# robocin/rSoccer

Measured on AMD Instinct MI355X. Metric: env-steps/sec (whole node), VSS-v0 3v3 @4096 envs, 1/2/4/8 GPU + CPU ref, higher is better.
Workload: dtype f32

## Files before the change

### __graft_entry__.py

```python
import os
import subprocess
import sys

ROOT = os.path.dirname(os.path.abspath(__file__))
if ROOT not in sys.path:
    sys.path.insert(0, ROOT)

CSRC = os.path.join(ROOT, "rsoccer_amd", "csrc")
HIP_SO = os.path.join(ROOT, "rsoccer_amd", "librsx_hip.so")
HIPCC_COMMON = ["--offload-arch=gfx950", "-O3", "-std=c++17", "-ffp-contract=off", "-fPIC",
                "-Wno-unused-value",
                "-mllvm", "-amdgpu-kernarg-preload-count=12",
                "-I" + os.path.join(ROOT, "include"), "-I" + CSRC]
HIP_UNITS = [
    ("rsx_api.hip", []),
    ("rsx_api_task.hip", []),
    ("rsx_api_ext.hip", []),
    ("rsx_lanes.hip", ["-mllvm", "-amdgpu-sched-strategy=max-ilp"]),
    ("rsx_epl.hip", ["-fno-slp-vectorize"]),
    ("rsx_big.hip", ["-fno-slp-vectorize"]),
    ("rsx_phys.hip", ["-mllvm", "-amdgpu-sched-strategy=max-ilp"]),
    ("rsx_sysid.hip", ["-mllvm", "-amdgpu-sched-strategy=max-ilp"]),
    ("rsx_plan.hip", ["-fno-slp-vectorize"]),
    ("rsx_plan_sampled.hip", ["-fno-slp-vectorize"]),
    ("rsx_policy.hip", ["-fno-slp-vectorize"]),
    ("rsx_render.hip", []),
    ("rsx_xfer.hip", []),
]

def _stale(target, sources):
    if not os.path.exists(target):
        return True
    t = os.path.getmtime(target)
# ... 79 lines not shown
```

### include/rsx.h

```cpp
#ifndef RSX_H
#define RSX_H

#include <stddef.h>
#include <stdint.h>

#ifdef __cplusplus
extern "C" {
#endif

#define RSX_ABI_VERSION 6
#define RSX_PHYSICS_MODEL 2

#define RSX_KIND_VSS 0
#define RSX_KIND_SSL 1

#define RSX_TASK_NONE                 0
#define RSX_TASK_VSS_V0               1
#define RSX_TASK_SSL_STATIC_DEFENDERS 2
#define RSX_TASK_SSL_DRIBBLING        3
#define RSX_TASK_SSL_CONTESTED        4
#define RSX_TASK_SSL_PASS_ENDURANCE   5
#define RSX_TASK_SSL_SCRIMMAGE         6
#define RSX_TASK_SSL_SCRIMMAGE_CROWDED 7

// ... 67 lines not shown
int rsx_step_dev(rsx_sim* h, void* stream);

int rsx_step_dev_flip(rsx_sim* h, void* stream);
int rsx_state_buffers(rsx_sim* h, float** current, float** other);
int rsx_reset_dev(rsx_sim* h, const float* ball_dev, const float* blue_dev, const float* yellow_dev,
                  const uint8_t* env_mask_dev, void* stream);

int rsx_step_dev_random(rsx_sim* h, int n, uint64_t seed, uint32_t first_tick, void* stream);


int rsx_task_attach(rsx_sim* h, int task, uint64_t seed, uint64_t env_id_base,
                    int max_episode_steps);
int rsx_task_view_get(rsx_sim* h, rsx_task_view* out);
int rsx_task_reseed(rsx_sim* h, uint64_t seed, void* stream);
int rsx_task_layout(rsx_sim* h, char* out, size_t n);
int rsx_task_placement_cache_stats(rsx_sim* h, int64_t out[2], void* stream);

int rsx_task_reset(rsx_sim* h, void* stream);
int rsx_task_reset_to(rsx_sim* h, const double* ball, const double* blue, const double* yellow,
                      const uint8_t* env_mask, void* stream);

int rsx_task_step(rsx_sim* h, const float* actions_dev, void* stream);
int rsx_task_step_n(rsx_sim* h, int n, void* stream);
int rsx_task_rollout(rsx_sim* h, int n, void* stream);

int rsx_task_enable_capture(rsx_sim* h, void* stream);
int rsx_drop_pending_hip_error(void);
int rsx_task_tick(rsx_sim* h, uint32_t* out, void* stream);

int rsx_task_lookahead(rsx_sim* h, const float* actions_dev, int n_candidates, int horizon, float gamma,
// ... 90 lines not shown
```

### rsoccer_amd/_lib.py

```python
import ctypes as C
import os

import numpy as np

_HERE = os.path.dirname(os.path.abspath(__file__))
LIB_PATH = os.environ.get("RSX_LIB") or os.path.join(_HERE, "librsx_hip.so")

KIND_VSS, KIND_SSL = 0, 1
TASK_NONE, TASK_VSS_V0, TASK_SSL_STATIC_DEFENDERS = 0, 1, 2
TASK_SSL_DRIBBLING, TASK_SSL_CONTESTED, TASK_SSL_PASS_ENDURANCE = 3, 4, 5
TASK_SSL_SCRIMMAGE, TASK_SSL_SCRIMMAGE_CROWDED = 6, 7
FIELD_KEYS = (
    "length", "width", "penalty_length", "penalty_width", "goal_width", "goal_depth",
    "ball_radius", "rbt_distance_center_kicker", "rbt_kicker_thickness", "rbt_kicker_width",
    "rbt_wheel0_angle", "rbt_wheel1_angle", "rbt_wheel2_angle", "rbt_wheel3_angle",
    "rbt_radius", "rbt_wheel_radius", "rbt_motor_max_rpm",
)
N_METRICS = 8
X_ROWS = 2
PHYSICS_PARAMS = ("m_robot", "m_ball", "e_rr", "e_rb", "e_wb", "e_wr", "mu_rr", "mu_rb", "mu_wb", "mu_g", "spin_dec",
                  "a_lin", "a_ang", "a_lat")
PHYSICS_COEFS = ("w_rb_r", "w_rb_b", "kt_rb_r", "kt_rb_b", "ope_rr", "ope_rb", "ope_wb", "e_wb", "e_wr", "mu_rr", "mu_rb", "mu_wb",
                 "a_lin_h", "a_lin_h2", "a_lat_h", "a_ang_h", "mu_g_dt", "spin_dec_dt")
PHYS_RAW, PHYS_COEF = 0, 1
TRACE_TERMS = ("ball_xy", "ball_v", "robot_xy", "robot_heading", "robot_v", "robot_omega")
METRIC_NAMES = ("env_steps", "episodes", "goals_for", "goals_against", "return_sum_q20",
                "episode_len_sum", "truncated_episodes", "reserved")

SYMBOLS = (
    "rsx_abi_version", "rsx_last_error", "rsx_device_count", "rsx_create", "rsx_destroy",
    "rsx_get_field_params", "rsx_reset", "rsx_step", "rsx_get_state", "rsx_step_state", "rsx_wire_buffers", "rsx_step_wire", "rsx_set_state",
    "rsx_get_state_full", "rsx_dev_view_get", "rsx_step_dev", "rsx_step_dev_random", "rsx_step_dev_flip", "rsx_state_buffers",
    "rsx_reset_dev", "rsx_task_attach",
    "rsx_task_view_get", "rsx_task_reseed", "rsx_task_layout", "rsx_task_placement_cache_stats", "rsx_task_reset", "rsx_task_reset_to", "rsx_task_step",
    "rsx_task_step_n", "rsx_task_rollout", "rsx_read_metrics", "rsx_metrics_fold", "rsx_check_finite",
    "rsx_task_checkpoint_size", "rsx_task_checkpoint_save", "rsx_task_checkpoint_load",
    "rsx_task_enable_capture", "rsx_task_tick", "rsx_drop_pending_hip_error", "rsx_task_lookahead",
    "rsx_physics_defaults", "rsx_physics_derive", "rsx_physics_enable", "rsx_physics_set", "rsx_physics_get",
    "rsx_physics_randomize", "rsx_physics_errors",
    "rsx_trace_load", "rsx_trace_eval",
    "rsx_render_view_reference", "rsx_render_size", "rsx_render_field", "rsx_render_open", "rsx_render", "rsx_render_errors",
    "rsx_task_transfer", "rsx_task_transfer_errors",
    "rsx_task_lookahead_sampled", "rsx_plan_candidates", "rsx_plan_update",
    "rsx_policy_num_params", "rsx_task_lookahead_policy",
)
ACT_RELU, ACT_TANH, ACT_CLIP = 0, 1, 2


class RsxError(RuntimeError):
# ... 54 lines not shown
    try:
        import torch
    except Exception:
        pass
    lib = C.CDLL(LIB_PATH)
    lib.rsx_last_error.restype = C.c_char_p
    vp, ip, dp = C.c_void_p, C.c_int, C.POINTER(C.c_double)
    lib.rsx_create.argtypes = [C.POINTER(vp), ip, ip, ip, ip, ip, ip, ip]
    lib.rsx_destroy.argtypes = [vp]
    lib.rsx_get_field_params.argtypes = [vp, dp]
    lib.rsx_reset.argtypes = [vp, vp, vp, vp, vp, vp]
    lib.rsx_step.argtypes = [vp, vp, vp]
    lib.rsx_get_state.argtypes = [vp, vp, vp]
    lib.rsx_step_state.argtypes = [vp, vp, vp, vp]
    lib.rsx_task_layout.argtypes = [vp, C.c_char_p, C.c_size_t]
    lib.rsx_task_placement_cache_stats.argtypes = [vp, C.POINTER(C.c_int64), vp]
    lib.rsx_set_state.argtypes = [vp, vp, vp]
    lib.rsx_wire_buffers.argtypes = [vp, C.POINTER(vp), C.POINTER(vp)]
    lib.rsx_step_wire.argtypes = [vp, vp]
    lib.rsx_get_state_full.argtypes = [vp, vp, vp]
    lib.rsx_dev_view_get.argtypes = [vp, C.POINTER(DevView)]
    lib.rsx_step_dev.argtypes = [vp, vp]
    lib.rsx_step_dev_random.argtypes = [vp, ip, C.c_uint64, C.c_uint32, vp]
    lib.rsx_step_dev_flip.argtypes = [vp, vp]
    lib.rsx_state_buffers.argtypes = [vp, C.POINTER(vp), C.POINTER(vp)]
    lib.rsx_reset_dev.argtypes = [vp, vp, vp, vp, vp, vp]
    lib.rsx_task_attach.argtypes = [vp, ip, C.c_uint64, C.c_uint64, ip]
    lib.rsx_task_view_get.argtypes = [vp, C.POINTER(TaskView)]
    lib.rsx_task_reseed.argtypes = [vp, C.c_uint64, vp]
    lib.rsx_task_reset.argtypes = [vp, vp]
# ... 229 lines not shown

    def task_attach(self, task, seed=0, env_id_base=0, max_episode_steps=0):
        _chk(self._lib.rsx_task_attach(self._h, task, seed, env_id_base, max_episode_steps))
        t = TaskView()
        _chk(self._lib.rsx_task_view_get(self._h, C.byref(t)))
        self._tview = t
        self.task = task
        self.obs_dim, self.act_dim, self.info_dim = t.obs_dim, t.act_dim, t.info_dim
        self.max_episode_steps = t.max_episode_steps

    def task_layout(self):
        buf = C.create_string_buffer(64)
        _chk(self._lib.rsx_task_layout(self._h, buf, 64))
        return buf.value.decode()

    def placement_cache_stats(self, stream=None):
        out = (C.c_int64 * 2)()
        _chk(self._lib.rsx_task_placement_cache_stats(self._h, out, self._stream(stream)))
        return int(out[0]), int(out[1])

    def task_tensors(self):
        t, B = self._tview, self.num_envs
        return dict(
            obs=self._tensor(t.obs, (B, t.obs_dim), "<f4"),
            reward=self._tensor(t.reward, (B,), "<f4"),
            terminated=self._tensor(t.terminated, (B,), "|u1"),
            truncated=self._tensor(t.truncated, (B,), "|u1"),
            info=self._rows(t.info, t.info_dim, t.row_stride),
            final_obs=self._tensor(t.final_obs, (B, t.obs_dim), "<f4"),
            steps=self._tensor(t.steps, (B,), "<i4"),
# ... 222 lines not shown
```

### rsoccer_amd/csrc/rsx_api_task.hip

```cpp
#include <cmath>
#include <cstdio>
#include <cstring>

#include "rsx_handle.hpp"
#include "rsx_math.hpp"
#include "rsx_plan_common.hpp"

using namespace rsx;

#ifndef RSX_PCACHE_MAX_ENVS
#define RSX_PCACHE_MAX_ENVS 16384
#endif

namespace {

int grid_for(const rsx_sim* h) { return lane_grid(h->L, h->P.num_envs); }
int helpers_for(const rsx_sim* h, int mode) { return mode == MODE_STEP && h->d_pcache && !h->d_phys ? (h->P.num_envs + 63) / 64 : 0; }

Layout stepping_layout(const rsx_sim* h, int mode) { return mode == MODE_STEP ? h->plan.step : mode == MODE_ROLLOUT ? h->plan.rollout : Layout::Lanes; }
int step_grid(const rsx_sim* h, int mode) {
    switch (stepping_layout(h, mode)) {
        case Layout::Epl: return epl_grid(h->P.num_envs);
        case Layout::Quad: return ssl_quad_grid(h->P.num_envs);
        default: return grid_for(h) + helpers_for(h, mode);
    }
}
void launch_task_of(const rsx_sim* h, const float* actions, int n_steps, int mode, hipStream_t s) {
    const Buffers b = buffers_of(h, mode == MODE_STEP ? actions : nullptr);
    const bool rollout = mode == MODE_ROLLOUT;
    switch (stepping_layout(h, mode)) {
        case Layout::Epl:
            if (h->P.task == RSX_TASK_VSS_V0) launch_vss_epl(rollout, h->P, b, n_steps, s); else launch_ssl_epl(h->P.task, rollout, h->P, b, n_steps, s);
            break;
        case Layout::Quad: launch_ssl_quad(h->P, b, n_steps, s); break;
        case Layout::LanesBig: launch_scrimmage_big(rollout, h->P, b, n_steps, s); break;
        case Layout::Lanes:
            if (h->d_phys) launch_task_phys(h->P, b, h->L, h->NR, h->d_phys, n_steps, mode, s);
            else launch_task(h->P, b, h->L, h->NR, helpers_for(h, mode), n_steps, mode, s);
            break;
    }
}
bool rollout_as_steps(const rsx_sim* h) { return h->plan.rollout_as_steps || (h->tick_dev && h->plan.step == Layout::Quad); }

}

void rsx::plan_stepping(rsx_sim* h) {
    const Params& P = h->P;
    h->plan = plan_layout(LayoutQuery{P.task, P.kind, h->L, h->NR, P.n_blue, P.num_envs, P.row_stride, P.state_dim, P.obs_dim, P.n_sub,
                                      h->d_phys != nullptr, std::getenv("RSX_LAYOUT")});
    h->tick_slots = step_grid(h, MODE_STEP);
}

extern "C" {

int rsx_task_attach(rsx_sim* h, int task, uint64_t seed, uint64_t env_id_base, int max_episode_steps) {
    RSX_ENTER(h);
    if (h->P.task != RSX_TASK_NONE) return fail(RSX_ERR_STATE, "a task is already attached");
    if (env_id_base > 0xFFFFFFFFull || env_id_base + (uint64_t)h->P.num_envs > 0x100000000ull)
        return fail(RSX_ERR_ARG, "env_id_base + num_envs exceeds 2^32 (global env ids are 32-bit)");
    Params P = h->P;
    if (derive_task(task, seed, env_id_base, max_episode_steps, h->M, P))
        return fail(RSX_ERR_ARG, "task does not match the simulator (VSS_V0: VSS, n_blue >= 1; STATIC_DEFENDERS: SSL 1vN; DRIBBLING: SSL 1v4; CONTESTED: SSL 1v1; PASS_ENDURANCE: SSL 2v0; SCRIMMAGE: SSL)");
    if (P.obs_dim > 64) return fail(RSX_ERR_ARG, "observation wider than 64 floats is not supported");
    if (task >= RSX_TASK_SSL_DRIBBLING && task <= RSX_TASK_SSL_PASS_ENDURANCE && h->L != 8)
// ... 89 lines not shown
    HIP_TRY(hipMemcpyAsync(out, h->d_pcstats, 2 * sizeof(int64_t), hipMemcpyDeviceToHost, (hipStream_t)stream));
    HIP_TRY(hipStreamSynchronize((hipStream_t)stream));
    return RSX_OK;
}

int rsx_task_layout(rsx_sim* h, char* out, size_t n) {
    if (!h || !out || n == 0) return fail(RSX_ERR_ARG, "null argument");
    if (h->P.task == RSX_TASK_NONE) return fail(RSX_ERR_STATE, "no task attached (rsx_task_attach)");
    const Layout lay = h->plan.step;
    const char* name = lay == Layout::Epl ? "one-lane-per-env" : lay == Layout::Quad ? "four-lanes-per-env" : lay == Layout::LanesBig ? "32-lanes-per-env-large-batch"
                     : h->L == 8 ? "8-lanes-per-env" : h->L == 16 ? "16-lanes-per-env" : h->L == 32 ? "32-lanes-per-env" : "64-lanes-per-env";
    std::snprintf(out, n, "%s", name);
    return RSX_OK;
}

int rsx_task_view_get(rsx_sim* h, rsx_task_view* out) {
    if (!h || !out) return fail(RSX_ERR_ARG, "null argument");
    if (h->P.task == RSX_TASK_NONE) return fail(RSX_ERR_STATE, "no task attached (rsx_task_attach)");
    const size_t B = (size_t)h->P.num_envs;
    out->task = h->P.task; out->obs_dim = h->P.obs_dim; out->act_dim = h->M.act_dim;
    out->info_dim = h->M.info_dim; out->max_episode_steps = h->P.max_steps;
    const size_t S = (size_t)h->P.row_stride;
    out->obs = h->d_obs; out->reward = h->d_aux + (size_t)ROW_REWARD * S;
    out->terminated = h->d_flags; out->truncated = h->d_flags + B;
    out->info = h->d_aux + (size_t)ROW_INFO * S; out->final_obs = h->d_final_obs;
    out->steps = (int32_t*)(h->d_aux + (size_t)ROW_STEPS * S); out->actions = h->d_actions;
    out->metrics = (int64_t*)h->d_metrics; out->row_stride = h->P.row_stride;
    return RSX_OK;
}

// ... 424 lines not shown
```

### rsoccer_amd/csrc/rsx_layout.hpp

```cpp
#pragma once
#include <algorithm>
#include <cstddef>
#include <cstring>

#include "rsx.h"
#include "rsx_params.hpp"

#ifndef RSX_EPL_MIN_ENVS
#define RSX_EPL_MIN_ENVS 98304
#endif
#ifndef RSX_EPL_MIN_ENVS_SSL
#define RSX_EPL_MIN_ENVS_SSL 65536
#endif
constexpr int RSX_EPL_MIN_ENVS_DRIBBLING = 49152, RSX_EPL_MIN_ENVS_DUEL = 32768;
#ifndef RSX_BIG_MIN_ENVS
#define RSX_BIG_MIN_ENVS 8192
#endif
#ifndef RSX_QUAD_MIN_ENVS
#define RSX_QUAD_MIN_ENVS 32768
#endif
#ifndef RSX_QUAD_MIN_ENVS_CROWDED
#define RSX_QUAD_MIN_ENVS_CROWDED 65536
#endif
#ifndef RSX_QUAD_ROLLOUT_MIN_ENVS
#define RSX_QUAD_ROLLOUT_MIN_ENVS 49152
#endif
#ifndef RSX_QUAD_ROLLOUT_MIN_ENVS_CROWDED
#define RSX_QUAD_ROLLOUT_MIN_ENVS_CROWDED 196608
#endif

namespace rsx {

enum class Layout { Lanes, LanesBig, Quad, Epl };

struct StepPlan {
    Layout step = Layout::Lanes;
    Layout rollout = Layout::Lanes;
    bool rollout_as_steps = false;
};

struct LayoutQuery {
    int task, kind, L, NR, n_blue, num_envs, row_stride, state_dim, obs_dim, n_sub;
    bool physics;
    const char* env_layout;
};

inline StepPlan plan_layout(const LayoutQuery& q) {
    StepPlan p;
    if (q.physics) return p;
    const auto asked = [&](const char* name) { return q.env_layout && std::strcmp(q.env_layout, name) == 0; };
    const int task = q.task, n_robots = (q.state_dim - 5) / (q.kind == RSX_KIND_VSS ? ModelD<RSX_KIND_VSS>::rs : ModelD<RSX_KIND_SSL>::rs);
    const size_t rows = (size_t)std::max(q.state_dim + X_ROWS, aux_rows(n_robots));
    const bool rows_below_2g = rows * (size_t)q.row_stride * sizeof(float) < ((size_t)1 << 31);
    if ((task == RSX_TASK_SSL_SCRIMMAGE || task == RSX_TASK_SSL_SCRIMMAGE_CROWDED) && q.NR == 22 && q.L == 32) {
        const bool spread = task == RSX_TASK_SSL_SCRIMMAGE;
        p.step = p.rollout = q.num_envs >= RSX_BIG_MIN_ENVS ? Layout::LanesBig : Layout::Lanes;
        const int quad_min = spread ? RSX_QUAD_MIN_ENVS : RSX_QUAD_MIN_ENVS_CROWDED;
        const bool fits = rows_below_2g && q.n_sub > 0 && q.n_blue == 11;
        if (fits && (q.env_layout ? asked("quad") : (quad_min > 0 && q.num_envs >= quad_min))) {
            p.step = Layout::Quad;
            p.rollout_as_steps = q.num_envs >= (spread ? RSX_QUAD_ROLLOUT_MIN_ENVS : RSX_QUAD_ROLLOUT_MIN_ENVS_CROWDED);
        }
        return p;
    }
    const bool fixed_ssl = task == RSX_TASK_SSL_DRIBBLING || task == RSX_TASK_SSL_CONTESTED || task == RSX_TASK_SSL_PASS_ENDURANCE;
    if ((task == RSX_TASK_VSS_V0 && q.NR == 6 && q.L == 8) || (task == RSX_TASK_SSL_STATIC_DEFENDERS && q.NR == 7 && q.L == 8) || fixed_ssl) {
        const int epl_min = task == RSX_TASK_VSS_V0 ? RSX_EPL_MIN_ENVS : task == RSX_TASK_SSL_STATIC_DEFENDERS ? RSX_EPL_MIN_ENVS_SSL
                          : task == RSX_TASK_SSL_DRIBBLING ? RSX_EPL_MIN_ENVS_DRIBBLING : RSX_EPL_MIN_ENVS_DUEL;
        const bool epl = asked("epl") || (!asked("lanes") && q.num_envs >= epl_min);
        if (epl && rows_below_2g && (size_t)q.num_envs * q.obs_dim * sizeof(float) < ((size_t)1 << 31)) p.step = p.rollout = Layout::Epl;
    }
    return p;
}

}
```

### rsoccer_amd/csrc/rsx_task_step_body.inc

```
    constexpr bool HOT = MODE != MODE_ROLLOUT;
    Params P = P_;
    Buffers bufs = bufs_;
    if (HOT) {
        RSX_UNPACK_HOT(P);
        bufs.state = hp_state; bufs.aux = hp_aux; bufs.actions = hp_in; bufs.flags = hp_flags;
    }
    const int n_steps_arg = hp_n_steps & RSX_N_STEPS_MASK;
    constexpr int mode = MODE == MODE_ROLLOUT ? MODE_STEP : MODE;
    const int n_steps = MODE == MODE_ROLLOUT ? n_steps_arg : 1;
    const bool tick_dev = __builtin_expect((hp_n_steps & RSX_TICK_DEV) != 0, 0);
    using K = KC<KIND>;
    using T = TC<TASK>;
    constexpr int G = 64 / L;
    constexpr int ID = T::info_dim;
    constexpr int AD = T::act_dim;
    __shared__ Shared<L> sh;
    constexpr bool PC = !PHYS && MODE == MODE_STEP && L == 8 && TASK == RSX_TASK_SSL_STATIC_DEFENDERS && NR == 7;
    if constexpr (PC) {
        if (__builtin_expect(bufs.pcache != nullptr && (int)blockIdx.x >= hp_per_xcd * 8, 0)) {
            const StepTick th = step_tick(tick_dev, P, bufs, 1u);
            if (th.ok) placement_helper<KIND, L, TASK, (PC ? NR : 1)>(P, bufs, (int)blockIdx.x - hp_per_xcd * 8, th.t, sh);
            return;
        }
    }
    StepTick tk{0u, true};
    if (MODE == MODE_STEP || MODE == MODE_ROLLOUT) {
        tk = step_tick(tick_dev, P, bufs, (uint32_t)n_steps);
        if (__builtin_expect(!tk.ok, 0)) return;
    }
    const uint32_t tick0 = tk.t;
    const int lane = threadIdx.x;
    const int b = LaneMap<L>::body(lane), g = LaneMap<L>::env(lane);
    const int tile = tile_of_block(HOT ? hp_per_xcd : (int)(gridDim.x >> 3));
    const int e = tile * G + g;
    const int N = NR ? NR : P.n_robots;
    const bool live = e < P.num_envs;
    const bool is_robot = live && b < N, is_ball = live && b == N;
    const size_t B = (size_t)P.num_envs;
    const uint32_t env_id = P.env_id_base + (uint32_t)e;
    constexpr int OD_C = obs_dim_c<TASK, NR>();
    const int OD = OD_C ? OD_C : P.obs_dim;
#define auxe(ROW) at_byte(bufs.aux, (ix_t)(ROW) * ((ix_t)4 * (ix_t)P.row_stride) + (ix_t)4 * (ix_t)e)

#ifdef RSX_TIMING
    if (lane == 0) { sh.dbg = bufs.dbg; bufs.dbg[(size_t)13 * gridDim.x + blockIdx.x] = __builtin_amdgcn_s_memrealtime(); }
#endif
    RSX_STAMP(0);
    Body o; float od, wd, wheels[4];
    const RawBody raw = load_raw<KIND>(P, bufs.state, e, b, is_robot, is_ball);
    constexpr bool CODE_PF = !PHYS && KIND == RSX_KIND_VSS && MODE == MODE_STEP;
    uint32_t code_touch = 0;
    if (CODE_PF) {
        unsigned long long pc;
        asm volatile("s_getpc_b64 %0" : "=s"(pc));
        code_touch = __builtin_nontemporal_load(reinterpret_cast<const uint32_t*>(reinterpret_cast<const char*>(pc) + 128u * (unsigned)lane));
    }
    std::conditional_t<PHYS, EnvCoef, LitCoef<KIND>> cf{};
    if constexpr (PHYS) if (live) load_coefs(P, phys, e, cf);
    int steps = 0; uint32_t episode = 0;
    if (live) {
        steps = __float_as_int(auxe(ROW_STEPS));
        episode = __float_as_uint(auxe(ROW_EPISODE));
    }
    float ou0 = 0.0f, ou1 = 0.0f;
    if (TASK == RSX_TASK_VSS_V0 && is_robot && b >= 1) {
        ou0 = auxe(ROW_OU + 2 * b); ou1 = auxe(ROW_OU + 2 * b + 1);
    }
    float info[10] = {0, 0, 0, 0, 0, 0, 0, 0, 0, 0};
    float prev_pot = 0.0f, ep_ret = 0.0f;
    if (is_ball) {
#pragma unroll
        for (int i = 0; i < ID; ++i)
            if (!(TASK == RSX_TASK_VSS_V0 && (i == 0 || i >= 4))) info[i] = auxe(ROW_INFO + i);
        prev_pot = auxe(ROW_PREV_POT);
        if (TASK != RSX_TASK_VSS_V0) ep_ret = auxe(ROW_EP_RET);
    }
    const bool counts_steps = (MODE == MODE_STEP || MODE == MODE_ROLLOUT) && blockIdx.x == 0 && lane == 0;
    unsigned long long steps_before = 0;
    if (counts_steps) steps_before = bufs.metrics[0];
    float reward = 0.0f; int term = 0, trunc = 0;
    bool success = false;
    bool against = false;
    bool was_reset = false;
    const bool fed = MODE == MODE_STEP && bufs.actions != nullptr;
    float act[AD];
#pragma unroll
    for (int i = 0; i < AD; ++i) act[i] = 0.0f;
    if (TASK == RSX_TASK_SSL_SCRIMMAGE) {
        if (fed && is_robot) {
#pragma unroll
            for (int i = 0; i < AD; ++i) act[i] = at_byte(bufs.actions, (ix_t)4 * (((ix_t)e * (ix_t)N + (ix_t)b) * (ix_t)AD + (ix_t)i));
// ... 5 lines not shown

    float pcx = 0.0f, pcy = 0.0f, pcth = 0.0f;
    uint32_t ptag = 0u;
    bool pc_on = false;
    if constexpr (PC) {
        pc_on = bufs.pcache != nullptr;
        if (pc_on && (is_robot || is_ball)) {
            constexpr int NBD = (PC ? NR : 1) + 1;
            const float* const pr = bufs.pcache + (size_t)((tick0 + 1u) & 1u) * (size_t)pcache_rows<NBD>() * B;
            pcx = pr[(size_t)(0 * NBD + b) * B + e]; pcy = pr[(size_t)(1 * NBD + b) * B + e]; pcth = pr[(size_t)(2 * NBD + b) * B + e];
            ptag = __float_as_uint(pr[(size_t)(3 * NBD) * B + e]);
        }
    }

    StepDraw pre;
    if (MODE == MODE_STEP) pre = draw_for_step<KIND, TASK>(P, env_id, tick0, b, is_robot, fed);

    __builtin_amdgcn_s_waitcnt(0x0F70);
    if (CODE_PF) asm volatile("" :: "v"(code_touch));
    interpret_body<KIND>(raw, is_robot, is_ball, o, od, wd, wheels);
    RSX_STAMP(1);

    for (int it = 0; it < n_steps; ++it) {
        bool ended;
        const float obs_ts = prev_pot;
        if (mode == 2) {
            const bool flagged = live && bufs.flags[2 * B + e] != 0;
            if (flagged) {
                episode += 1; steps = 0; ou0 = 0.0f; ou1 = 0.0f;
                if constexpr (PHYS) phys_redraw(P, phys, e, env_id, episode, b == 0, cf);
                if (is_ball) {
#pragma unroll
                    for (int i = 0; i < 10; ++i) info[i] = 0.0f;
#pragma unroll
                    for (int i = 0; i < ID; ++i) auxe(ROW_INFO + i) = 0.0f;
// ... 31 lines not shown
            physics<KIND, L, NR>(P, o, b, g, live, sh, cf);
            RSX_STAMP(3);
            if (MODE == MODE_STEP && KIND == RSX_KIND_SSL) {
                typedef const __attribute__((address_space(4))) uint32_t* kw_t;
                constexpr size_t KOFF = RSX_PARAMS_KERNARG_OFFSET;
                static_assert(sizeof(Params) % 4 == 0 && KOFF % 4 == 0, "parameter block in dwords");
                kw_t pk = (kw_t)__builtin_amdgcn_kernarg_segment_ptr() + KOFF / 4;
                asm volatile("" : "+s"(pk));
                struct Words { uint32_t w[sizeof(Params) / 4]; } raw;
#pragma unroll
                for (size_t i = 0; i < sizeof(Params) / 4; ++i) raw.w[i] = pk[i];
                P = __builtin_bit_cast(Params, raw);
                RSX_UNPACK_HOT(P);
            }

#include "rsx_step_wire.inc"
            write_obs<KIND, TASK>(P, bufs.obs + (size_t)e * OD, b, is_robot, is_ball, o.x, o.y, o.vx, o.vy, o.s, o.c, wd, o.ir, obs_ts);
#include "rsx_step_xr.inc"
            wave_sync();
            if (is_ball) {
                const float* xr = sh.x0[g];
                task_reward<KIND, TASK>(P, xr, o.x, o.y, lastx, lasty, first_step, prev_pot, info, reward, term, success, against);
                ep_ret = ep_ret + reward;
            }
            steps += 1;
            trunc = steps >= P.max_steps;
            const unsigned long long endm = __ballot(is_ball && (term | trunc));
            ended = live && ((endm >> (LaneMap<L>::slot(N, g))) & 1ull) != 0;
            if (is_ball) {
#pragma unroll
                for (int i = 0; i < ID; ++i)
                    if (!(TASK == RSX_TASK_VSS_V0 && (i == 0 || i >= 4)) || term || first_step) auxe(ROW_INFO + i) = info[i];
                auxe(ROW_REWARD) = reward;
                if (MODE == MODE_STEP) { bufs.flags[(ix_t)e] = (uint8_t)term; bufs.flags[(ix_t)P.num_envs + (ix_t)e] = (uint8_t)trunc; }
                else { bufs.flags[e] = (uint8_t)term; bufs.flags[B + e] = (uint8_t)trunc; }
            }
        }

        RSX_STAMP(4);
        if (RSX_RARE_B(KIND, 4, __any(ended))) {
            if (ended && mode == 0) {
                write_obs<KIND, TASK>(P, bufs.final_obs + (size_t)e * OD, b, is_robot, is_ball, o.x, o.y, o.vx, o.vy, o.s, o.c, wd, o.ir, obs_ts);
            }
            if (ended && mode == 0) episode += 1;
            if (KIND == RSX_KIND_VSS) {
                if (ended && is_ball && mode == 0) {
                    unsigned long long* const ms = metric_slot(bufs);
                    atomicAdd(&ms[1], 1ull);
                    if (info[4] > 0.0f) atomicAdd(&ms[2], 1ull);
                    if (info[5] > 0.0f) atomicAdd(&ms[3], 1ull);
                    atomicAdd(&ms[4], (unsigned long long)__float2ll_rn(vss_episode_return(info) * 1048576.0f));
                    atomicAdd(&ms[5], (unsigned long long)steps);
                    if (trunc && !term) atomicAdd(&ms[6], 1ull);
                }
            } else if (mode == 0) {
                static_assert(KIND == RSX_KIND_VSS || L >= 6, "metrics fan-out needs 6 lanes per env");
                uint32_t* const mv = reinterpret_cast<uint32_t*>(sh.x0[g]);
                if (ended && is_ball) {
                    unsigned long long inc[6];
                    inc[0] = 1ull;
                    inc[1] = success ? 1ull : 0ull;
                    inc[2] = against ? 1ull : 0ull;
                    inc[3] = (unsigned long long)__float2ll_rn(ep_ret * 1048576.0f);
                    inc[4] = (unsigned long long)steps;
                    inc[5] = (trunc && !term) ? 1ull : 0ull;
#pragma unroll
                    for (int k = 0; k < 6; ++k) { mv[2 * k] = (uint32_t)inc[k]; mv[2 * k + 1] = (uint32_t)(inc[k] >> 32); }
                }
                wave_sync();
// ... 47 lines not shown
            RSX_STAMP(18);
        }

        wave_sync();
    }

    RSX_STAMP(5);
    if (mode != 2) store_body<KIND>(P, bufs.state, e, b, is_robot, is_ball, o, od, wd, wheels, P.n_sub != 0 || was_reset);
    if (live && b == 0) {
        auxe(ROW_STEPS) = __int_as_float(steps);
        auxe(ROW_EPISODE) = __uint_as_float(episode);
    }
    if (TASK == RSX_TASK_VSS_V0 && is_robot && b >= 1) {
        auxe(ROW_OU + 2 * b) = ou0; auxe(ROW_OU + 2 * b + 1) = ou1;
    }
    if (is_ball) {
        auxe(ROW_PREV_POT) = prev_pot;
        if (TASK != RSX_TASK_VSS_V0) auxe(ROW_EP_RET) = ep_ret;
#undef auxe
    }
    if (counts_steps) bufs.metrics[0] = steps_before + (unsigned long long)P.num_envs * (unsigned long long)n_steps;
    RSX_STAMP(6);
#ifdef RSX_TIMING
    __builtin_amdgcn_s_waitcnt(0x0F70);
    RSX_STAMP(7);
    if (lane == 0) bufs.dbg[(size_t)14 * gridDim.x + blockIdx.x] = __builtin_amdgcn_s_memrealtime();
#endif
```

### rsoccer_amd/csrc/rsx_units.hpp

```cpp
#pragma once
#include <hip/hip_runtime.h>

#include <cstdint>

struct rsx_render_view;

namespace rsx {

struct Params;
struct Buffers;

void launch_sim(const Params& P, const Buffers& b, int L, int NR, float* state_out, int rand_tick, hipStream_t s);
void launch_task(const Params& P, const Buffers& b, int L, int NR, int helpers, int n_steps, int mode, hipStream_t s);
void launch_count_nonfinite(const float* p, size_t n, unsigned long long* out, hipStream_t s);
void launch_fold_metrics(unsigned long long* metrics, unsigned long long* slots, hipStream_t s);
void launch_reset_dev(float* st, const float* ball, const float* blue, const float* yellow, const uint8_t* mask, int B, int S, int rows,
                      int rs, int nb, int ny, float r_ball, hipStream_t s);
void launch_wire_cmds_in(const double* wire, float* cmds, unsigned B, unsigned NC, unsigned S, hipStream_t s);
void launch_wire_state_out(const float* st, double* wire, unsigned B, unsigned rows, unsigned S, hipStream_t s);
void launch_tick_fill(uint32_t* slots, int from, int to, uint32_t value, int copy, hipStream_t s);
#ifdef RSX_TIMING
inline unsigned long long* g_dbg = nullptr;
#endif
void launch_vss_epl(bool rollout, const Params& P, const Buffers& b, int n_steps, hipStream_t s);
void launch_ssl_epl(int task, bool rollout, const Params& P, const Buffers& b, int n_steps, hipStream_t s);
void launch_ssl_quad(const Params& P, const Buffers& b, int n_steps, hipStream_t s);
int epl_grid(int num_envs);
int ssl_quad_grid(int num_envs);
void launch_scrimmage_big(bool rollout, const Params& P, const Buffers& b, int n_steps, hipStream_t s);
void launch_task_phys(const Params& P, const Buffers& b, int L, int NR, float* phys, int n_steps, int mode, hipStream_t s);
void launch_sim_phys(const Params& P, const Buffers& b, int L, int NR, float* phys, float* state_out, int rand_tick, hipStream_t s);
void launch_phys_init(float* blk, int B, int S, int kind, int ts_ms, hipStream_t s);
void launch_phys_set(float* blk, const float* vals, const uint8_t* mask, int B, int S, int vstride, hipStream_t s);
void launch_phys_ranges(float* blk, const float* lo, const float* hi, uint32_t mask, hipStream_t s);
void launch_trace_eval(const Params& P, int L, int NR, const float* phys, float* state, float* loss, const float* frames,
                       const float* cmds, const int32_t* anchors, int n_frames, int n_anchors, int horizon, hipStream_t s);
long long lookahead_grid(int L, int num_envs, int n_candidates);
void launch_task_lookahead(const Params& P, int L, int NR, const float* state, const float* aux, const uint32_t* ticks, const float* phys,
                           const float* actions, int n_candidates, int horizon, float gamma, float* returns, int32_t* steps,
                           uint8_t* flags, float* last_obs, hipStream_t s);
struct PlanSampler;
void launch_task_lookahead_sampled(const Params& P, int L, int NR, const float* state, const float* aux, const uint32_t* ticks, const float* phys,
                                   const float* mean, const PlanSampler& S, int n_candidates, int horizon, float gamma, float* returns,
                                   int32_t* steps, uint8_t* flags, float* last_obs, hipStream_t s);
// ... 25 lines not shown
```

### rsoccer_amd/csrc/rsx_variants.hpp

```cpp
#pragma once
#include <type_traits>
#include <utility>

#include "rsx_launch.hpp"
#include "rsx_kernels.hpp"

namespace rsx {

template <int V> using int_c = std::integral_constant<int, V>;


template <int MAX_L, typename F>
void with_generic_variant(const int L, F&& f) {
    static_assert(MAX_L == 32 || MAX_L == 64, "widest lane group the unit instantiates");
    switch (L) {
        case 8: f(int_c<8>{}, int_c<0>{}); break;
        case 16: f(int_c<16>{}, int_c<0>{}); break;
        case 32: f(int_c<32>{}, int_c<0>{}); break;
        default: f(int_c<MAX_L>{}, int_c<0>{}); break;
    }
}

template <int KIND, int MAX_L, typename F>
void with_sim_variant(const int L, const int NR, F&& f) {
// ... 34 lines not shown
template <typename F>
void with_mode(const int mode, F&& f) {
    switch (mode) {
        case MODE_STEP: f(int_c<MODE_STEP>{}); break;
        case MODE_ROLLOUT: f(int_c<MODE_ROLLOUT>{}); break;
        case MODE_RESET: f(int_c<MODE_RESET>{}); break;
        default: f(int_c<MODE_REFRESH>{}); break;
    }
}
inline int mode_steps(const int mode, const int n_steps) { return mode == MODE_STEP || mode == MODE_ROLLOUT ? n_steps : 1; }

struct HotGrid {
    int tiles, helpers = 0;
    size_t lds = 0;
    int per_xcd = 0;
};

template <typename... KArgs, typename... Tail>
void launch_hot(void (*kernel)(KArgs...), const HotGrid& g, hipStream_t s, float* out, const float* in, const int n, const Params& P,
                const Buffers& b, Tail&&... tail) {
    rsx_launch(kernel, dim3((unsigned)(g.tiles + g.helpers)), dim3(64), g.lds, s, b.state, out, in, b.flags, P.num_envs,
               RSX_HOT_DIM(P.state_dim, P.row_stride, P.num_envs), g.per_xcd ? g.per_xcd : g.tiles >> 3, n, P, b, std::forward<Tail>(tail)...);
}
template <typename... KArgs, typename... Tail>
void launch_task_hot(void (*kernel)(KArgs...), const HotGrid& g, hipStream_t s, const int n_steps, const Params& P, const Buffers& b, Tail&&... tail) {
    launch_hot(kernel, g, s, b.aux, b.actions, n_steps, P, b, std::forward<Tail>(tail)...);
}
template <typename... KArgs, typename... Tail>
void launch_sim_hot(void (*kernel)(KArgs...), const HotGrid& g, hipStream_t s, float* state_out, const int rand_tick, const Params& P, const Buffers& b, Tail&&... tail) {
    launch_hot(kernel, g, s, state_out, b.cmds, rand_tick, P, b, std::forward<Tail>(tail)...);
}

}
```

Baseline: 436.2 million.

## Split VSS-v0 single step into paired physics and service wavefronts

Adds a 128-thread paired kernel for the VSS-v0 single-step path at small env counts. The second wavefront loads episode bookkeeping, draws the random actions, and later computes reward, flags and metrics from ball positions passed through LDS. The first wavefront runs physics and obs writes. The aim is to take the RNG draws, aux loads and reward tail off the critical physics wavefront, at the cost of LDS traffic and workgroup barriers.

New measurement: 448.9 million, median of 6. 1.03x the previous value.

```diff
diff --git a/__graft_entry__.py b/__graft_entry__.py
--- a/__graft_entry__.py
+++ b/__graft_entry__.py
@@ -17,6 +17,7 @@
     ("rsx_api_task.hip", []),
     ("rsx_api_ext.hip", []),
     ("rsx_lanes.hip", ["-mllvm", "-amdgpu-sched-strategy=max-ilp"]),
+    ("rsx_pair.hip", ["-mllvm", "-amdgpu-sched-strategy=max-ilp"]),
     ("rsx_epl.hip", ["-fno-slp-vectorize"]),
     ("rsx_big.hip", ["-fno-slp-vectorize"]),
     ("rsx_phys.hip", ["-mllvm", "-amdgpu-sched-strategy=max-ilp"]),
diff --git a/include/rsx.h b/include/rsx.h
--- a/include/rsx.h
+++ b/include/rsx.h
@@ -105,6 +105,7 @@
 int rsx_task_view_get(rsx_sim* h, rsx_task_view* out);
 int rsx_task_reseed(rsx_sim* h, uint64_t seed, void* stream);
 int rsx_task_layout(rsx_sim* h, char* out, size_t n);
+int rsx_task_service_wave(rsx_sim* h, int* out);
 int rsx_task_placement_cache_stats(rsx_sim* h, int64_t out[2], void* stream);
 
 int rsx_task_reset(rsx_sim* h, void* stream);
diff --git a/rsoccer_amd/_lib.py b/rsoccer_amd/_lib.py
--- a/rsoccer_amd/_lib.py
+++ b/rsoccer_amd/_lib.py
@@ -32,7 +32,7 @@
     "rsx_get_field_params", "rsx_reset", "rsx_step", "rsx_get_state", "rsx_step_state", "rsx_wire_buffers", "rsx_step_wire", "rsx_set_state",
     "rsx_get_state_full", "rsx_dev_view_get", "rsx_step_dev", "rsx_step_dev_random", "rsx_step_dev_flip", "rsx_state_buffers",
     "rsx_reset_dev", "rsx_task_attach",
-    "rsx_task_view_get", "rsx_task_reseed", "rsx_task_layout", "rsx_task_placement_cache_stats", "rsx_task_reset", "rsx_task_reset_to", "rsx_task_step",
+    "rsx_task_view_get", "rsx_task_reseed", "rsx_task_layout", "rsx_task_service_wave", "rsx_task_placement_cache_stats", "rsx_task_reset", "rsx_task_reset_to", "rsx_task_step",
     "rsx_task_step_n", "rsx_task_rollout", "rsx_read_metrics", "rsx_metrics_fold", "rsx_check_finite",
     "rsx_task_checkpoint_size", "rsx_task_checkpoint_save", "rsx_task_checkpoint_load",
     "rsx_task_enable_capture", "rsx_task_tick", "rsx_drop_pending_hip_error", "rsx_task_lookahead",
@@ -117,6 +117,7 @@
     lib.rsx_get_state.argtypes = [vp, vp, vp]
     lib.rsx_step_state.argtypes = [vp, vp, vp, vp]
     lib.rsx_task_layout.argtypes = [vp, C.c_char_p, C.c_size_t]
+    lib.rsx_task_service_wave.argtypes = [vp, C.POINTER(C.c_int)]
     lib.rsx_task_placement_cache_stats.argtypes = [vp, C.POINTER(C.c_int64), vp]
     lib.rsx_set_state.argtypes = [vp, vp, vp]
     lib.rsx_wire_buffers.argtypes = [vp, C.POINTER(vp), C.POINTER(vp)]
@@ -376,6 +377,11 @@
         _chk(self._lib.rsx_task_layout(self._h, buf, 64))
         return buf.value.decode()
 
+    def task_service_wave(self):
+        out = C.c_int(0)
+        _chk(self._lib.rsx_task_service_wave(self._h, C.byref(out)))
+        return bool(out.value)
+
     def placement_cache_stats(self, stream=None):
         out = (C.c_int64 * 2)()
         _chk(self._lib.rsx_task_placement_cache_stats(self._h, out, self._stream(stream)))
diff --git a/rsoccer_amd/csrc/rsx_api_task.hip b/rsoccer_amd/csrc/rsx_api_task.hip
--- a/rsoccer_amd/csrc/rsx_api_task.hip
+++ b/rsoccer_amd/csrc/rsx_api_task.hip
@@ -36,6 +36,7 @@
         case Layout::LanesBig: launch_scrimmage_big(rollout, h->P, b, n_steps, s); break;
         case Layout::Lanes:
             if (h->d_phys) launch_task_phys(h->P, b, h->L, h->NR, h->d_phys, n_steps, mode, s);
+            else if (mode == MODE_STEP && h->plan.service_wave) launch_task_pair(h->P, b, n_steps, s);
             else launch_task(h->P, b, h->L, h->NR, helpers_for(h, mode), n_steps, mode, s);
             break;
     }
@@ -47,7 +48,7 @@
 void rsx::plan_stepping(rsx_sim* h) {
     const Params& P = h->P;
     h->plan = plan_layout(LayoutQuery{P.task, P.kind, h->L, h->NR, P.n_blue, P.num_envs, P.row_stride, P.state_dim, P.obs_dim, P.n_sub,
-                                      h->d_phys != nullptr, std::getenv("RSX_LAYOUT")});
+                                      h->d_phys != nullptr, std::getenv("RSX_LAYOUT"), std::getenv("RSX_SERVICE_WAVE")});
     h->tick_slots = step_grid(h, MODE_STEP);
 }
 
@@ -167,6 +168,13 @@
     return RSX_OK;
 }
 
+int rsx_task_service_wave(rsx_sim* h, int* out) {
+    if (!h || !out) return fail(RSX_ERR_ARG, "null argument");
+    if (h->P.task == RSX_TASK_NONE) return fail(RSX_ERR_STATE, "no task attached (rsx_task_attach)");
+    *out = h->plan.step == Layout::Lanes && h->plan.service_wave && !h->d_phys ? 1 : 0;
+    return RSX_OK;
+}
+
 int rsx_task_view_get(rsx_sim* h, rsx_task_view* out) {
     if (!h || !out) return fail(RSX_ERR_ARG, "null argument");
     if (h->P.task == RSX_TASK_NONE) return fail(RSX_ERR_STATE, "no task attached (rsx_task_attach)");
diff --git a/rsoccer_amd/csrc/rsx_layout.hpp b/rsoccer_amd/csrc/rsx_layout.hpp
--- a/rsoccer_amd/csrc/rsx_layout.hpp
+++ b/rsoccer_amd/csrc/rsx_layout.hpp
@@ -28,6 +28,9 @@
 #ifndef RSX_QUAD_ROLLOUT_MIN_ENVS_CROWDED
 #define RSX_QUAD_ROLLOUT_MIN_ENVS_CROWDED 196608
 #endif
+#ifndef RSX_SERVICE_WAVE_MAX_ENVS
+#define RSX_SERVICE_WAVE_MAX_ENVS 4096
+#endif
 
 namespace rsx {
 
@@ -37,12 +40,14 @@
     Layout step = Layout::Lanes;
     Layout rollout = Layout::Lanes;
     bool rollout_as_steps = false;
+    bool service_wave = false;
 };
 
 struct LayoutQuery {
     int task, kind, L, NR, n_blue, num_envs, row_stride, state_dim, obs_dim, n_sub;
     bool physics;
     const char* env_layout;
+    const char* env_service;
 };
 
 inline StepPlan plan_layout(const LayoutQuery& q) {
@@ -70,6 +75,8 @@
         const bool epl = asked("epl") || (!asked("lanes") && q.num_envs >= epl_min);
         if (epl && rows_below_2g && (size_t)q.num_envs * q.obs_dim * sizeof(float) < ((size_t)1 << 31)) p.step = p.rollout = Layout::Epl;
     }
+    if (task == RSX_TASK_VSS_V0 && q.NR == 6 && q.L == 8 && p.step == Layout::Lanes)
+        p.service_wave = q.env_service ? std::strcmp(q.env_service, "1") == 0 : q.num_envs <= RSX_SERVICE_WAVE_MAX_ENVS;
     return p;
 }
 
diff --git a/rsoccer_amd/csrc/rsx_pair.hip b/rsoccer_amd/csrc/rsx_pair.hip
--- /dev/null
+++ b/rsoccer_amd/csrc/rsx_pair.hip
@@ -0,0 +1,16 @@
+#include <hip/hip_runtime.h>
+
+#include "rsx.h"
+#include "rsx_units.hpp"
+#include "rsx_variants.hpp"
+#include "rsx_pair.hpp"
+
+namespace rsx {
+
+void launch_task_pair(const Params& P, const Buffers& b, int n_steps, hipStream_t s) {
+    HotGrid g{lane_grid(8, P.num_envs)};
+    g.threads = 128;
+    launch_task_hot((task_pair_step_kernel<RSX_KIND_VSS, 8, RSX_TASK_VSS_V0, 6, MODE_STEP>), g, s, n_steps, P, b);
+}
+
+}
diff --git a/rsoccer_amd/csrc/rsx_pair.hpp b/rsoccer_amd/csrc/rsx_pair.hpp
--- /dev/null
+++ b/rsoccer_amd/csrc/rsx_pair.hpp
@@ -0,0 +1,29 @@
+#pragma once
+#include "rsx_kernels.hpp"
+
+namespace rsx {
+
+struct PairBox {
+    float2 dr[64];
+    float4 ball[8];
+    uint32_t tick;
+    uint32_t ok;
+};
+
+__device__ __forceinline__ void pair_barrier() {
+    __builtin_amdgcn_fence(__ATOMIC_RELEASE, "workgroup", "local");
+    __builtin_amdgcn_s_barrier();
+    __builtin_amdgcn_fence(__ATOMIC_ACQUIRE, "workgroup", "local");
+}
+
+template <int KIND, int L, int TASK, int NR, int MODE>
+__global__ __launch_bounds__(128) void task_pair_step_kernel(RSX_HOT_ARGS, const Params P_, const Buffers bufs_) {
+    static_assert(KIND == RSX_KIND_VSS && TASK == RSX_TASK_VSS_V0 && L == 8 && MODE == MODE_STEP, "the paired form exists for the VSS-v0 single step");
+    constexpr bool PHYS = false;
+    float* const phys = nullptr;
+#define RSX_STEP_PAIRED 1
+#include "rsx_task_step_body.inc"
+#undef RSX_STEP_PAIRED
+}
+
+}
diff --git a/rsoccer_amd/csrc/rsx_step_ball_load.inc b/rsoccer_amd/csrc/rsx_step_ball_load.inc
--- /dev/null
+++ b/rsoccer_amd/csrc/rsx_step_ball_load.inc
@@ -0,0 +1,7 @@
+    if (is_ball) {
+#pragma unroll
+        for (int i = 0; i < ID; ++i)
+            if (!(TASK == RSX_TASK_VSS_V0 && (i == 0 || i >= 4))) info[i] = auxe(ROW_INFO + i);
+        prev_pot = auxe(ROW_PREV_POT);
+        if (TASK != RSX_TASK_VSS_V0) ep_ret = auxe(ROW_EP_RET);
+    }
diff --git a/rsoccer_amd/csrc/rsx_step_pair_tail.inc b/rsoccer_amd/csrc/rsx_step_pair_tail.inc
--- /dev/null
+++ b/rsoccer_amd/csrc/rsx_step_pair_tail.inc
@@ -0,0 +1,11 @@
+#include "rsx_step_xr.inc"
+            if (is_ball) pb.ball[g] = make_float4(o.x, o.y, lastx, lasty);
+            RSX_STAMP(23);
+            pair_barrier();
+            term = is_ball && (o.x > P.half_len || o.x < -P.half_len);
+            steps += 1;
+            trunc = steps >= P.max_steps;
+            const unsigned long long endm = __ballot(is_ball && (term | trunc));
+            ended = live && ((endm >> (LaneMap<L>::slot(N, g))) & 1ull) != 0;
+#include "rsx_step_wire.inc"
+            write_obs<KIND, TASK>(P, bufs.obs + (size_t)e * OD, b, is_robot, is_ball, o.x, o.y, o.vx, o.vy, o.s, o.c, wd, o.ir, obs_ts);
diff --git a/rsoccer_amd/csrc/rsx_step_reward.inc b/rsoccer_amd/csrc/rsx_step_reward.inc
--- /dev/null
+++ b/rsoccer_amd/csrc/rsx_step_reward.inc
@@ -0,0 +1,17 @@
+            if (is_ball) {
+                const float* xr = sh.x0[g];
+                task_reward<KIND, TASK>(P, xr, o.x, o.y, lastx, lasty, first_step, prev_pot, info, reward, term, success, against);
+                ep_ret = ep_ret + reward;
+            }
+            steps += 1;
+            trunc = steps >= P.max_steps;
+            const unsigned long long endm = __ballot(is_ball && (term | trunc));
+            ended = live && ((endm >> (LaneMap<L>::slot(N, g))) & 1ull) != 0;
+            if (is_ball) {
+#pragma unroll
+                for (int i = 0; i < ID; ++i)
+                    if (!(TASK == RSX_TASK_VSS_V0 && (i == 0 || i >= 4)) || term || first_step) auxe(ROW_INFO + i) = info[i];
+                auxe(ROW_REWARD) = reward;
+                if (MODE == MODE_STEP) { bufs.flags[(ix_t)e] = (uint8_t)term; bufs.flags[(ix_t)P.num_envs + (ix_t)e] = (uint8_t)trunc; }
+                else { bufs.flags[e] = (uint8_t)term; bufs.flags[B + e] = (uint8_t)trunc; }
+            }
diff --git a/rsoccer_amd/csrc/rsx_step_service.inc b/rsoccer_amd/csrc/rsx_step_service.inc
--- /dev/null
+++ b/rsoccer_amd/csrc/rsx_step_service.inc
@@ -0,0 +1,35 @@
+    {
+        float info[10] = {0, 0, 0, 0, 0, 0, 0, 0, 0, 0};
+        float prev_pot = 0.0f, ep_ret = 0.0f;
+#include "rsx_step_ball_load.inc"
+        int steps = 0;
+        if (is_ball) steps = __float_as_int(auxe(ROW_STEPS));
+        const uint32_t code_touch = __builtin_nontemporal_load(reinterpret_cast<const uint32_t*>(reinterpret_cast<const char*>(code_pc) + 128u * (unsigned)lane));
+        const bool fed = bufs.actions != nullptr;
+        const StepDraw dr = draw_for_step<KIND, TASK>(P, env_id, tick0, b, is_robot, fed);
+        pb.dr[lane] = make_float2(dr.v[0], dr.v[1]);
+        __builtin_amdgcn_s_waitcnt(0x0F70);
+        asm volatile("" :: "v"(code_touch));
+        RSX_STAMP(19);
+        pair_barrier();
+
+        pair_barrier();
+        RSX_STAMP(20);
+        float reward = 0.0f; int term = 0, trunc = 0;
+        bool success = false, against = false, ended;
+        const bool first_step = steps == 0;
+        if (first_step) {
+#pragma unroll
+            for (int i = 0; i < 10; ++i) info[i] = 0.0f;
+        }
+        const float4 bl = pb.ball[g];
+        const struct { float x, y; } o = {bl.x, bl.y};
+        const float lastx = bl.z, lasty = bl.w;
+#include "rsx_step_reward.inc"
+        if (__any(ended)) {
+#include "rsx_step_vss_metrics.inc"
+        }
+        if (is_ball) auxe(ROW_PREV_POT) = prev_pot;
+        RSX_STAMP(21);
+        return;
+    }
diff --git a/rsoccer_amd/csrc/rsx_step_vss_metrics.inc b/rsoccer_amd/csrc/rsx_step_vss_metrics.inc
--- /dev/null
+++ b/rsoccer_amd/csrc/rsx_step_vss_metrics.inc
@@ -0,0 +1,9 @@
+                if (ended && is_ball && mode == 0) {
+                    unsigned long long* const ms = metric_slot(bufs);
+                    atomicAdd(&ms[1], 1ull);
+                    if (info[4] > 0.0f) atomicAdd(&ms[2], 1ull);
+                    if (info[5] > 0.0f) atomicAdd(&ms[3], 1ull);
+                    atomicAdd(&ms[4], (unsigned long long)__float2ll_rn(vss_episode_return(info) * 1048576.0f));
+                    atomicAdd(&ms[5], (unsigned long long)steps);
+                    if (trunc && !term) atomicAdd(&ms[6], 1ull);
+                }
diff --git a/rsoccer_amd/csrc/rsx_task_step_body.inc b/rsoccer_amd/csrc/rsx_task_step_body.inc
--- a/rsoccer_amd/csrc/rsx_task_step_body.inc
+++ b/rsoccer_amd/csrc/rsx_task_step_body.inc
@@ -24,12 +24,32 @@
         }
     }
     StepTick tk{0u, true};
+#ifdef RSX_STEP_PAIRED
+    __shared__ PairBox pb;
+    const int wv = __builtin_amdgcn_readfirstlane((int)(threadIdx.x >> 6));
+    unsigned long long code_pc;
+    asm volatile("s_getpc_b64 %0" : "=s"(code_pc));
+    if (tick_dev) {
+        if (wv == 0) {
+            tk = step_tick(true, P, bufs, 1u);
+            if (threadIdx.x == 0) { pb.tick = tk.t; pb.ok = tk.ok ? 1u : 0u; }
+        }
+        pair_barrier();
+        if (wv != 0) tk = StepTick{(uint32_t)__builtin_amdgcn_readfirstlane((int)pb.tick), __builtin_amdgcn_readfirstlane((int)pb.ok) != 0};
+    } else {
+        tk = step_tick(false, P, bufs, 1u);
+    }
+    if (__builtin_expect(!tk.ok, 0)) return;
+    const uint32_t tick0 = tk.t;
+    const int lane = threadIdx.x & 63;
+#else
     if (MODE == MODE_STEP || MODE == MODE_ROLLOUT) {
         tk = step_tick(tick_dev, P, bufs, (uint32_t)n_steps);
         if (__builtin_expect(!tk.ok, 0)) return;
     }
     const uint32_t tick0 = tk.t;
     const int lane = threadIdx.x;
+#endif
     const int b = LaneMap<L>::body(lane), g = LaneMap<L>::env(lane);
     const int tile = tile_of_block(HOT ? hp_per_xcd : (int)(gridDim.x >> 3));
     const int e = tile * G + g;
@@ -41,6 +61,10 @@
     constexpr int OD_C = obs_dim_c<TASK, NR>();
     const int OD = OD_C ? OD_C : P.obs_dim;
 #define auxe(ROW) at_byte(bufs.aux, (ix_t)(ROW) * ((ix_t)4 * (ix_t)P.row_stride) + (ix_t)4 * (ix_t)e)
+#ifdef RSX_STEP_PAIRED
+    if (wv != 0)
+#include "rsx_step_service.inc"
+#endif
 
 #ifdef RSX_TIMING
     if (lane == 0) { sh.dbg = bufs.dbg; bufs.dbg[(size_t)13 * gridDim.x + blockIdx.x] = __builtin_amdgcn_s_memrealtime(); }
@@ -48,7 +72,11 @@
     RSX_STAMP(0);
     Body o; float od, wd, wheels[4];
     const RawBody raw = load_raw<KIND>(P, bufs.state, e, b, is_robot, is_ball);
+#ifdef RSX_STEP_PAIRED
+    constexpr bool CODE_PF = false;
+#else
     constexpr bool CODE_PF = !PHYS && KIND == RSX_KIND_VSS && MODE == MODE_STEP;
+#endif
     uint32_t code_touch = 0;
     if (CODE_PF) {
         unsigned long long pc;
@@ -68,13 +96,9 @@
     }
     float info[10] = {0, 0, 0, 0, 0, 0, 0, 0, 0, 0};
     float prev_pot = 0.0f, ep_ret = 0.0f;
-    if (is_ball) {
-#pragma unroll
-        for (int i = 0; i < ID; ++i)
-            if (!(TASK == RSX_TASK_VSS_V0 && (i == 0 || i >= 4))) info[i] = auxe(ROW_INFO + i);
-        prev_pot = auxe(ROW_PREV_POT);
-        if (TASK != RSX_TASK_VSS_V0) ep_ret = auxe(ROW_EP_RET);
-    }
+#ifndef RSX_STEP_PAIRED
+#include "rsx_step_ball_load.inc"
+#endif
     const bool counts_steps = (MODE == MODE_STEP || MODE == MODE_ROLLOUT) && blockIdx.x == 0 && lane == 0;
     unsigned long long steps_before = 0;
     if (counts_steps) steps_before = bufs.metrics[0];
@@ -110,11 +134,23 @@
     }
 
     StepDraw pre;
+#ifndef RSX_STEP_PAIRED
     if (MODE == MODE_STEP) pre = draw_for_step<KIND, TASK>(P, env_id, tick0, b, is_robot, fed);
+#endif
 
     __builtin_amdgcn_s_waitcnt(0x0F70);
     if (CODE_PF) asm volatile("" :: "v"(code_touch));
     interpret_body<KIND>(raw, is_robot, is_ball, o, od, wd, wheels);
+#ifdef RSX_STEP_PAIRED
+    RSX_STAMP(22);
+    pair_barrier();
+    {
+        const float2 d2 = pb.dr[lane];
+#pragma unroll
+        for (int i = 0; i < 5; ++i) pre.v[i] = 0.0f;
+        pre.v[0] = d2.x; pre.v[1] = d2.y;
+    }
+#endif
     RSX_STAMP(1);
 
     for (int it = 0; it < n_steps; ++it) {
@@ -176,27 +212,15 @@
                 RSX_UNPACK_HOT(P);
             }
 
+#ifdef RSX_STEP_PAIRED
+#include "rsx_step_pair_tail.inc"
+#else
 #include "rsx_step_wire.inc"
             write_obs<KIND, TASK>(P, bufs.obs + (size_t)e * OD, b, is_robot, is_ball, o.x, o.y, o.vx, o.vy, o.s, o.c, wd, o.ir, obs_ts);
 #include "rsx_step_xr.inc"
             wave_sync();
-            if (is_ball) {
-                const float* xr = sh.x0[g];
-                task_reward<KIND, TASK>(P, xr, o.x, o.y, lastx, lasty, first_step, prev_pot, info, reward, term, success, against);
-                ep_ret = ep_ret + reward;
-            }
-            steps += 1;
-            trunc = steps >= P.max_steps;
-            const unsigned long long endm = __ballot(is_ball && (term | trunc));
-            ended = live && ((endm >> (LaneMap<L>::slot(N, g))) & 1ull) != 0;
-            if (is_ball) {
-#pragma unroll
-                for (int i = 0; i < ID; ++i)
-                    if (!(TASK == RSX_TASK_VSS_V0 && (i == 0 || i >= 4)) || term || first_step) auxe(ROW_INFO + i) = info[i];
-                auxe(ROW_REWARD) = reward;
-                if (MODE == MODE_STEP) { bufs.flags[(ix_t)e] = (uint8_t)term; bufs.flags[(ix_t)P.num_envs + (ix_t)e] = (uint8_t)trunc; }
-                else { bufs.flags[e] = (uint8_t)term; bufs.flags[B + e] = (uint8_t)trunc; }
-            }
+#include "rsx_step_reward.inc"
+#endif
         }
 
         RSX_STAMP(4);
@@ -206,15 +230,9 @@
             }
             if (ended && mode == 0) episode += 1;
             if (KIND == RSX_KIND_VSS) {
-                if (ended && is_ball && mode == 0) {
-                    unsigned long long* const ms = metric_slot(bufs);
-                    atomicAdd(&ms[1], 1ull);
-                    if (info[4] > 0.0f) atomicAdd(&ms[2], 1ull);
-                    if (info[5] > 0.0f) atomicAdd(&ms[3], 1ull);
-                    atomicAdd(&ms[4], (unsigned long long)__float2ll_rn(vss_episode_return(info) * 1048576.0f));
-                    atomicAdd(&ms[5], (unsigned long long)steps);
-                    if (trunc && !term) atomicAdd(&ms[6], 1ull);
-                }
+#ifndef RSX_STEP_PAIRED
+#include "rsx_step_vss_metrics.inc"
+#endif
             } else if (mode == 0) {
                 static_assert(KIND == RSX_KIND_VSS || L >= 6, "metrics fan-out needs 6 lanes per env");
                 uint32_t* const mv = reinterpret_cast<uint32_t*>(sh.x0[g]);
@@ -292,11 +310,13 @@
     if (TASK == RSX_TASK_VSS_V0 && is_robot && b >= 1) {
         auxe(ROW_OU + 2 * b) = ou0; auxe(ROW_OU + 2 * b + 1) = ou1;
     }
+#ifndef RSX_STEP_PAIRED
     if (is_ball) {
         auxe(ROW_PREV_POT) = prev_pot;
         if (TASK != RSX_TASK_VSS_V0) auxe(ROW_EP_RET) = ep_ret;
+    }
+#endif
 #undef auxe
-    }
     if (counts_steps) bufs.metrics[0] = steps_before + (unsigned long long)P.num_envs * (unsigned long long)n_steps;
     RSX_STAMP(6);
 #ifdef RSX_TIMING
diff --git a/rsoccer_amd/csrc/rsx_units.hpp b/rsoccer_amd/csrc/rsx_units.hpp
--- a/rsoccer_amd/csrc/rsx_units.hpp
+++ b/rsoccer_amd/csrc/rsx_units.hpp
@@ -28,6 +28,7 @@
 int epl_grid(int num_envs);
 int ssl_quad_grid(int num_envs);
 void launch_scrimmage_big(bool rollout, const Params& P, const Buffers& b, int n_steps, hipStream_t s);
+void launch_task_pair(const Params& P, const Buffers& b, int n_steps, hipStream_t s);
 void launch_task_phys(const Params& P, const Buffers& b, int L, int NR, float* phys, int n_steps, int mode, hipStream_t s);
 void launch_sim_phys(const Params& P, const Buffers& b, int L, int NR, float* phys, float* state_out, int rand_tick, hipStream_t s);
 void launch_phys_init(float* blk, int B, int S, int kind, int ts_ms, hipStream_t s);
diff --git a/rsoccer_amd/csrc/rsx_variants.hpp b/rsoccer_amd/csrc/rsx_variants.hpp
--- a/rsoccer_amd/csrc/rsx_variants.hpp
+++ b/rsoccer_amd/csrc/rsx_variants.hpp
@@ -72,12 +72,13 @@
     int tiles, helpers = 0;
     size_t lds = 0;
     int per_xcd = 0;
+    int threads = 64;
 };
 
 template <typename... KArgs, typename... Tail>
 void launch_hot(void (*kernel)(KArgs...), const HotGrid& g, hipStream_t s, float* out, const float* in, const int n, const Params& P,
                 const Buffers& b, Tail&&... tail) {
-    rsx_launch(kernel, dim3((unsigned)(g.tiles + g.helpers)), dim3(64), g.lds, s, b.state, out, in, b.flags, P.num_envs,
+    rsx_launch(kernel, dim3((unsigned)(g.tiles + g.helpers)), dim3((unsigned)g.threads), g.lds, s, b.state, out, in, b.flags, P.num_envs,
                RSX_HOT_DIM(P.state_dim, P.row_stride, P.num_envs), g.per_xcd ? g.per_xcd : g.tiles >> 3, n, P, b, std::forward<Tail>(tail)...);
 }
 template <typename... KArgs, typename... Tail>
```
